# Kmatsuo57/cell-image-analysis

Hardware: AMD Instinct MI355X
Metric: cells/sec screened (CAE fwd + recon-MSE + SVM score), 64x64 (higher is better)
Workload: dtype f32 (results in the fp32 error class; the contractions run as split 16-bit products on the matrix pipe, fp32 accumulate: conv1..conv6 as 2 fp16 terms x 3 products with exact power-of-two scales from each cell's own data, the PCA GEMM as 3 bf16 terms x 6 products, conv7's 32 -> 16 channel contraction; 1 GPU; BASELINE.json configs[2]: screening inference, 1000000 synthetic 64x64 crops on one GPU, resident in HBM, CAE fwd + recon MSE/MAE + RobustScaler + PCA(100) + 2x OCSVM score on device; cells_per_gpu=1000000, global_cells=1000000, chunk_cells=65536, detector_train_cells=5000, weights=random init (Glorot, non-trivial BN), seed 42, parallelism=dp1

## Files before the change

cell-image-analysis_amd/csrc/api.hip:

```cpp
#include "api_internal.hpp"
#include "tensor_archive.hpp"

using namespace cs;

static thread_local std::string g_err;

namespace cs {
int fail(int code, const char* fmt, ...)
{
    char buf[1024];
    va_list ap;
    va_start(ap, fmt);
    vsnprintf(buf, sizeof buf, fmt, ap);
    va_end(ap);
    g_err = buf;
    return code;
}
const char* last_error_cstr() { return g_err.c_str(); }
}

static const char* kKernelNames[K_COUNT] = {"conv1_relu_bn_pool", "conv2_relu_bn_pool", "conv3_relu_bn_pool",
                                            "conv4_relu_bn",      "conv5_up_relu_bn",   "conv6_up_relu_bn",
                                            "conv7_up_sigmoid_err", "scaler_pca",       "ocsvm_decision",
                                            "finalize",           "synth_crops",        "conv6_conv7_fused_err",
// ... 177 lines not shown
{
    std::vector<float> tmp;
    for (int l = 0; l < count; ++l) {
        const int cin = l == 0 ? 1 : kRefChannels[l - 1], cout = kRefChannels[l];
        const bool folded = (l == 4 || l == 5);
        const size_t nf = folded ? pack_conv_fragments_folded(cin, cout, nullptr, nullptr) : pack_conv_fragments(cin, cout, nullptr, nullptr);
        tmp.resize(nf);
        if (folded) pack_conv_fragments_folded(cin, cout, w->kernel[l], tmp.data());
        else pack_conv_fragments(cin, cout, w->kernel[l], tmp.data());
        int rc = upload(set.wfrag[l], tmp.data(), nf * sizeof(float));
        if (rc) return rc;
        std::vector<float> ep(3 * cout);
        for (int c = 0; c < cout; ++c) {
            const float s = w->bn_gamma[l][c] / sqrtf(w->bn_var[l][c] + w->bn_eps);
            ep[c] = w->bias[l][c];
            ep[cout + c] = s;
            ep[2 * cout + c] = w->bn_beta[l][c] - w->bn_mean[l][c] * s;
        }
        rc = upload(set.ep[l], ep.data(), ep.size() * sizeof(float));
        if (rc) return rc;
        if (l == 4 || l == 5) {
            tmp.resize(pack_wino_up_fragments(l, nullptr, nullptr));
            pack_wino_up_fragments(l, w->kernel[l], tmp.data());
            rc = upload(set.winoup[l], tmp.data(), tmp.size() * sizeof(float));
            if (rc) return rc;
        }
        if (l == 1 || l == 2) {
            tmp.resize(pack_wino_cs_fragments(l, nullptr, nullptr));
            pack_wino_cs_fragments(l, w->kernel[l], tmp.data());
            rc = upload(set.winocs[l], tmp.data(), tmp.size() * sizeof(float));
            if (rc) return rc;
        }
        if (l == 2) {
            std::vector<uint16_t> h2(pack_wino3_h2(nullptr, nullptr, nullptr));
            pack_wino3_h2(w->kernel[l], h2.data(), &set.c3h2_inv);
            rc = upload(set.c3h2, h2.data(), h2.size() * sizeof(uint16_t));
            if (rc) return rc;
        }
        if (l == 3) {
            std::vector<uint16_t> h2(pack_conv4_f16x2(nullptr, nullptr, nullptr));
            pack_conv4_f16x2(w->kernel[l], h2.data(), &set.c4h2_inv);
            rc = upload(set.c4h2, h2.data(), h2.size() * sizeof(uint16_t));
            if (rc) return rc;
        }
        if (l == 4) {
            std::vector<float> weff(pack_generic_folded(cin, cout, nullptr, nullptr));
            pack_generic_folded(cin, cout, w->kernel[l], weff.data());
            std::vector<uint16_t> h2(pack_conv5_f16x2(nullptr, nullptr, nullptr));
            pack_conv5_f16x2(weff.data(), h2.data(), &set.c5h2_inv);
            rc = upload(set.c5h2, h2.data(), h2.size() * sizeof(uint16_t));
            if (rc) return rc;
        }
        if (l == 5) {
            std::vector<float> weff(pack_generic_folded(cin, cout, nullptr, nullptr));
            pack_generic_folded(cin, cout, w->kernel[l], weff.data());
            std::vector<uint16_t> h2(pack_conv6_f16x2(nullptr, nullptr, nullptr));
            pack_conv6_f16x2(weff.data(), h2.data(), &set.c6h2_inv);
            rc = upload(set.c6h2, h2.data(), h2.size() * sizeof(uint16_t));
            if (rc) return rc;
        }
        if (l == 0) {
            tmp.resize(pack_conv12_conv1_fragments(nullptr, nullptr, nullptr));
            pack_conv12_conv1_fragments(w->kernel[l], ep.data() + cout, tmp.data());
            rc = upload(set.c12w1, tmp.data(), tmp.size() * sizeof(float));
            if (rc) return rc;
            pack_conv12_p1_bound(w->kernel[l], ep.data(), &set.p1a, &set.p1b);
            std::vector<unsigned int> wh(pack_conv12_conv1_h2(nullptr, nullptr, nullptr, nullptr));
            pack_conv12_conv1_h2(w->kernel[l], ep.data() + cout, wh.data(), &set.c12w1h2_inv);
            rc = upload(set.c12w1h2, wh.data(), wh.size() * sizeof(unsigned int));
            if (rc) return rc;
        }
        if (l == 1) {
            tmp.resize(pack_conv12_fragments(nullptr, nullptr, nullptr));
            pack_conv12_fragments(w->kernel[l], ep.data() + cout, tmp.data());
            rc = upload(set.c12, tmp.data(), tmp.size() * sizeof(float));
            if (rc) return rc;
            std::vector<unsigned int> uh(pack_conv12_fragments_h2(nullptr, nullptr, nullptr, nullptr));
            pack_conv12_fragments_h2(w->kernel[l], ep.data() + cout, uh.data(), &set.c12h2_inv);
            rc = upload(set.c12h2, uh.data(), uh.size() * sizeof(unsigned int));
            if (rc) return rc;
        }
    }
    set.n = count;
    return CS_OK;
}

static int pack_generic(GenSet& set, const cs_cae_weights* w, const Arch& a, int count, bool split16)
{
    for (int l = 0; l < count; ++l) {
        const int cin = a.cin(l), cout = a.ch[l];
        int rc = upload(set.w[l], w->kernel[l], sizeof(float) * 9 * cin * cout);
        if (rc) return rc;
        set.folded[l] = l > a.n_enc && ((l < a.n_conv - 1 && conv_generic_folds(a.gh[l], a.gw[l], cin, cout)) ||
                                        (l == a.n_conv - 1 && cout == 1 && cin % 4 == 0));
        if (set.folded[l]) {
            std::vector<float> wf(pack_generic_folded(cin, cout, nullptr, nullptr));
            pack_generic_folded(cin, cout, w->kernel[l], wf.data());
            if ((rc = upload(set.wf[l], wf.data(), wf.size() * sizeof(float)))) return rc;
            if (split16 && l == a.n_conv - 1 && cout == 1 && conv_last_x3_takes(a.gh[l], a.gw[l], cin)) {
                std::vector<uint16_t> pl(pack_last_bf16x3(cin, nullptr, nullptr));
                pack_last_bf16x3(cin, wf.data(), pl.data());
                if ((rc = upload(set.wx3[l], pl.data(), pl.size() * sizeof(uint16_t)))) return rc;
                set.x3[l] = true;
            }
            if (split16 && l < a.n_conv - 1 && conv_generic_x3_takes(a.gh[l], a.gw[l], cin, cout, 1)) {
                std::vector<uint16_t> pl(pack_generic_bf16x3(16, cin, cout, nullptr, nullptr));
                pack_generic_bf16x3(16, cin, cout, wf.data(), pl.data());
                if ((rc = upload(set.wx3[l], pl.data(), pl.size() * sizeof(uint16_t)))) return rc;
                set.x3[l] = true;
                std::vector<uint16_t> ph(pack_generic_f16x2(16, cin, cout, nullptr, nullptr, nullptr));
// ... 922 lines not shown
        else if (k == K_SCALER_PCA) per_cell = 2.0 * (double)m->F * m->C;
        else if (k == K_SVM) per_cell = 0.0;
        *flops = per_cell * (double)m->prof_cells[k];
    }
    return CS_OK;
}

int cs_profile_mfma_per_cell(cs_model* m, int k, double* mfma)
{
    if (!m || !mfma || k < 0 || k >= K_COUNT) return fail(CS_ERR_INVALID, "bad kernel id");
    double v = 0.0;
    if (k == K_SCALER_PCA) {
        *mfma = m->has_det && !m->split16 ? (double)m->fpad * m->cpad / 1024.0 : 0.0;
        return CS_OK;
    }
    if (m->arch.ref) {
        const bool h2 = m->split16;
        switch (k) {
            case K_CONV1: v = 1536; break;
            case K_CONV2: v = 8192; break;
            case K_CONV3: v = h2 ? 0 : 2048; break;
            case K_CONV4: v = h2 ? 0 : 576; break;
            case K_CONV5: v = h2 ? 0 : 1152; break;
            case K_CONV6: v = 4608; break;
            case K_CONV67_FUSED: v = h2 ? 512 : 4608 + 512; break;
            case K_CONV12_FUSED: v = h2 ? 0 : 4608 + 1536 + 48; break;
            default: v = 0.0;
        }
    } else if (k <= K_CONV6 || k == K_CONV7_ERR) {
        const int l = k == K_CONV7_ERR ? m->arch.n_conv - 1 : k - K_CONV1;
        if (l < m->arch.n_conv && !(m->split16 && m->gae.x3[l])) {
            const int cout_pad = (m->arch.ch[l] + 15) / 16 * 16;
            v = (double)m->arch.gh[l] * m->arch.gw[l] / 16.0 * (cout_pad / 16) * (9.0 * m->arch.cin(l) / 4.0);
        }
    }
    *mfma = v;
    return CS_OK;
}

int cs_profile_bf16_mfma_per_cell(cs_model* m, int k, double* mfma)
{
    if (!m || !mfma || k < 0 || k >= K_COUNT) return fail(CS_ERR_INVALID, "bad kernel id");
    double v = 0.0;
    if (!m->split16) { *mfma = 0.0; return CS_OK; }
    if (k == K_SCALER_PCA && m->has_det) {
        *mfma = (double)(m->cpad / 16) * (m->fpad / 32) * 6.0 / 16.0;
        return CS_OK;
    }
    if (m->arch.ref) {
        if (k == K_CONV4) v = 4 * 2 * 9 * 3;
        if (k == K_CONV3) v = 16.0 * 4 * 2 * 2 * 3;
        if (k == K_CONV12_FUSED) v = 66 * 8 * 2 + 36 * 4 * 4 * 3;
        if (k == K_CONV5) v = 4 * 4 * 4 * 4 * 3 + (m->fuse45 ? 4 * 2 * 9 * 3 : 0);
        if (k == K_CONV67_FUSED) v = 4.0 * 16 * 2 * 4 * 2 * 3;
    } else if (k <= K_CONV6) {
        const int l = k - K_CONV1;
        if (l < m->arch.n_conv && m->gae.x3[l]) {
            const int cout_pad = (m->arch.ch[l] + 15) / 16 * 16;
            const double taps = l > m->arch.n_enc ? 4.0 : 9.0;
            const bool last = l == m->arch.n_conv - 1;
            v = (double)m->arch.gh[l] * m->arch.gw[l] / 16.0 * (cout_pad / 16) * taps * (m->arch.cin(l) / 32.0) * ((m->gae.h2_inv[l] != 0.0f && !last) ? 3.0 : 6.0);
        }
    }
    *mfma = v;
    return CS_OK;
}

}
```

cell-image-analysis_amd/csrc/common.hpp:

```cpp
#pragma once
#include <hip/hip_runtime.h>
#include <stdint.h>
#include <stdio.h>

#include "../../include/cellscreen.h"

namespace cs {

typedef float f32x4 __attribute__((ext_vector_type(4)));

__device__ __forceinline__ unsigned int f16x2_split_word_scaled(float x, float S)
{
    unsigned int pk;
    asm("v_fma_mixlo_f16 %0, %1, %2, 0\n\t"
        "v_fma_mixhi_f16 %0, %1, %2, -%0 op_sel:[0,0,0] op_sel_hi:[0,0,1]"
        : "=&v"(pk) : "v"(x), "v"(S));
    return pk;
}
__device__ __forceinline__ void f16x2_split6_exchange(const float (&v)[6], unsigned int sel, unsigned int (&out)[6])
{
    unsigned int p0, p1, p2, p3, p4, p5;
    asm("v_cvt_f16_f32 %6, %12\n\t"
        "v_cvt_f16_f32 %7, %13\n\t"
        "v_cvt_f16_f32 %8, %14\n\t"
// ... 18 lines not shown
        "v_perm_b32 %3, %3, %9, %18\n\t"
        "v_perm_b32 %4, %4, %10, %18\n\t"
        "v_perm_b32 %5, %5, %11, %18"
        : "=&v"(out[0]), "=&v"(out[1]), "=&v"(out[2]), "=&v"(out[3]), "=&v"(out[4]), "=&v"(out[5]),
          "=&v"(p0), "=&v"(p1), "=&v"(p2), "=&v"(p3), "=&v"(p4), "=&v"(p5)
        : "v"(v[0]), "v"(v[1]), "v"(v[2]), "v"(v[3]), "v"(v[4]), "v"(v[5]), "v"(sel));
}

struct LayerGeom {
    int H, W, cin, cout;
    bool pool;
    bool ups;
    bool last;
};

enum KernelId {
    K_CONV1 = 0, K_CONV2, K_CONV3, K_CONV4, K_CONV5, K_CONV6, K_CONV7_ERR,
    K_SCALER_PCA, K_SVM, K_FINALIZE, K_SYNTH, K_CONV67_FUSED, K_CONV12_FUSED, K_COUNT
};

hipError_t launch_conv_mfma(int layer, const float* in, const float* wfrag, const float* ep,
                            float* out, int64_t n_cells, hipStream_t stream, bool folded = false);
size_t pack_conv_fragments_folded(int cin, int cout, const float* hwio, float* dst);
hipError_t launch_conv_wino_cs(int layer, const float* in, const float* ufrag, const float* ep, float* out, int64_t n_cells,
                               hipStream_t stream);
size_t pack_wino_cs_fragments(int layer, const float* hwio, float* dst);
hipError_t launch_conv3_wino_h2(const float* in, const uint16_t* uplanes, float inv_sw, const float* ep, float* out, int64_t n_cells,
                                hipStream_t stream);
size_t pack_wino3_h2(const float* hwio, uint16_t* dst, float* inv_sw);
hipError_t launch_conv12_fused(const float* x, const float* w1frag, const float* ep1, const float* ufrag, const float* ep2, float* p2,
                               int64_t n_cells, hipStream_t stream, const unsigned int* ufrag_h2 = nullptr,
                               float p1a = 0.0f, float p1b = 0.0f, float inv_sw = 1.0f, const unsigned int* w1h2 = nullptr, float inv_sw1 = 1.0f);
size_t pack_conv12_conv1_h2(const float* hwio, const float* bn_scale, unsigned int* dst, float* inv_sw1);
size_t pack_conv12_fragments_h2(const float* hwio, const float* bn_scale, unsigned int* dst, float* inv_sw);
void pack_conv12_p1_bound(const float* hwio1, const float* ep1, float* a1, float* b1);
size_t pack_conv12_fragments(const float* hwio, const float* bn_scale, float* dst);
size_t pack_conv12_conv1_fragments(const float* hwio, const float* bn_scale, float* dst);
hipError_t launch_conv4_h2(const float* in, const uint16_t* wfrag, float inv_sw, const float* ep, float* out, int64_t n_cells, hipStream_t stream);
size_t pack_conv4_f16x2(const float* hwio, uint16_t* dst, float* inv_sw);
hipError_t launch_conv5_h2(const float* in, const uint16_t* wfrag, float inv_sw, const float* ep, float* out, int64_t n_cells, hipStream_t stream);
hipError_t launch_conv45_h2(const float* in, const uint16_t* w4, float inv_sw4, const float* ep4, const uint16_t* w5, float inv_sw5,
                            const float* ep5, float* out, int64_t n_cells, hipStream_t stream);
size_t pack_conv5_f16x2(const float* weff, uint16_t* dst, float* inv_sw);
hipError_t launch_conv_wino_up(int layer, const float* in, const float* ufrag, const float* ep, float* out, int64_t n_cells,
                               hipStream_t stream);
size_t pack_wino_up_fragments(int layer, const float* hwio, float* dst);
size_t pack_conv_fragments(int cin, int cout, const float* hwio, float* dst);

hipError_t launch_conv67_fused(const float* a5, const float* ufrag, const float* ep, const float* x, const float* weff_dev,
                               const float* b7_dev, float* errpart, int64_t n_cells, hipStream_t stream);
int conv67_fused_nparts();
hipError_t launch_conv67_h2(const float* a5, const uint16_t* wplanes, float inv_sw, const float* ep, const float* x, const float* weff_dev,
                            const float* b7_dev, float* errpart, int64_t n_cells, hipStream_t stream);
size_t pack_conv6_f16x2(const float* weff, uint16_t* dst, float* inv_sw);
float f16x2_weight_scale(const float* w, size_t n);
void f16x2_split(float w, float S, uint16_t& hi, uint16_t& lo);

hipError_t launch_conv7_err(const float* a6, const float* x, const float* weff_dev, const float* b7_dev,
                            float* errpart, float* recon, int64_t n_cells, hipStream_t stream);
hipError_t launch_conv7_err_train(const float* a6, const float* x, const float* weff_dev, const float* b7_dev, float* errpart,
                                  float* recon, float* dz, float* dzsum_part, int64_t n_cells, hipStream_t stream);
void conv7_effective_weights(const float* w7_hwio, float* weff);

constexpr int TRAIN_MAX_PARTS = 256;
constexpr int BN_MAX_PARTS = 1024;
struct ReduceDesc { long dst; long len; const float* src; int nparts; long stride; };
hipError_t launch_conv_train_fwd(int layer, const float* in, const float* wfrag, const float* bias,
                                 float* relu_out, int64_t n_cells, hipStream_t stream, float* stats_part = nullptr,
                                 int* stats_parts = nullptr);
hipError_t launch_conv_dgrad(int layer, const float* dz, const float* wfrag_t, float* dx, int64_t n_cells,
                             hipStream_t stream);
hipError_t launch_bn_stats(const float* r, long P, int C, float* part, int* G, hipStream_t s);
hipError_t launch_bn_stats_final(const float* part, int G, int C, float eps, float momentum, float* mov_mean,
                                 float* mov_var, float* stats, hipStream_t s);
hipError_t launch_bn_stats_merge(const float* part, int G, int C, float* out , hipStream_t s);
hipError_t launch_bn_apply(const float* r, int C, const float* gamma, const float* beta, const float* stats, float* a,
                           long N, int H, int W, int pool, hipStream_t s);
hipError_t launch_loss_dz(const float* out, const float* y, long total, float* dz, float* dzsum_part, int* G, hipStream_t s,
                          const float* errpart = nullptr, long nparts = 0, float* out2 = nullptr);
hipError_t launch_loss_scalar(const float* errpart, long nparts, long nelem, float* out2, hipStream_t s);
hipError_t launch_bn_bwd_reduce(const float* da, const float* r, const float* stats, const float* gamma, const float* beta,
                                long N, int H, int W, int C, int pool, float* part, int* G, hipStream_t s);
hipError_t launch_bn_bwd_final(const float* part, int G, int C, double nred, float* sums, float* dgamma, float* dbeta,
                               hipStream_t s);
hipError_t launch_bn_bwd_dz(const float* da, const float* r, const float* stats, const float* gamma, const float* beta,
                            const float* sums, long N, int H, int W, int C, int pool, float* dz, float* dzsum_part,
                            int* Gz, hipStream_t s);
hipError_t launch_wgrad(int layer, const float* xin, const float* dz, float* part, int64_t n_cells, int* nparts,
                        hipStream_t s);
hipError_t launch_reduce_all(const ReduceDesc* descs_dev, int ndesc, long total_len, float* flat_grad, hipStream_t s,
                             const float* errpart = nullptr, long nparts = 0, long nelem = 0, float* out2 = nullptr);
hipError_t launch_adam(float* p, const float* g, float* m, float* v, long n, float alpha, float b1, float b2, float eps, hipStream_t s,
                       const float* batch_scal, double* macc);
enum { GEN_EPI_BN = 0, GEN_EPI_BN_POOL = 1, GEN_EPI_SIGMOID = 2, GEN_EPI_RELU = 3, GEN_EPI_PLAIN = 4 };
int conv_generic_supported(int H, int W, int cin, int cout, char* why, size_t why_len);
hipError_t launch_conv_generic(const float* in, const float* w_hwio, const float* ep, float* out, int64_t n, int H, int W, int cin,
                               int cout, int ups, int epi, hipStream_t stream, const float* w_folded = nullptr);
size_t pack_generic_folded(int cin, int cout, const float* hwio, float* dst);
int conv_generic_x3_takes(int H, int W, int cin, int cout, int ups);
size_t pack_generic_bf16x3(int ntaps, int cin, int cout, const float* w, uint16_t* dst);
hipError_t launch_pack_generic_bf16x3(const float* w, int ntaps, int cin, int cout, uint16_t* dst, hipStream_t stream);
hipError_t launch_conv_generic_x3(const float* in, const uint16_t* wplanes, const float* ep, float* out, int64_t n, int H, int W, int cin,
                                  int cout, int ups, int epi, hipStream_t stream, float inv_sw = 0.0f);
size_t pack_generic_f16x2(int ntaps, int cin, int cout, const float* w, uint16_t* dst, float* inv_sw);
int conv_last_x3_takes(int H, int W, int cin);
size_t pack_last_bf16x3(int cin, const float* weff, uint16_t* dst);
hipError_t launch_conv_last_x3(const float* in, const uint16_t* wplanes, const float* ep, float* out, int64_t n, int H, int W, int cin,
// ... 48 lines not shown
```

cell-image-analysis_amd/csrc/conv_wino_up.hip:

```cpp
#include "common.hpp"

#include <type_traits>

#include <cmath>
#include <cstdlib>
#include <cstring>

namespace cs {

namespace {

template <int HS_, int WS_, int CIN_, int COUT_>
struct WUCfg {
    static constexpr int HS = HS_, WS = WS_, CIN = CIN_, COUT = COUT_;
    static constexpr int HO = 2 * HS, WO = 2 * WS;
    static constexpr int TW = WS / 2;
    static constexpr int SR = 2 * (16 / TW);
    static constexpr int R = SR + 2, WP = WS + 2;
    static constexpr int PS = CIN + 4;
    static constexpr int STRIP = R * WP * PS * 4;
    static constexpr int LDS = 2 * STRIP;
    static constexpr int NGRP = HS / SR;
    static constexpr int NQ = CIN / 16, KS = CIN / 4;
    static constexpr int NSW = COUT / 32;
    static constexpr int NB = 9 * KS * NSW;
    static constexpr int C4 = CIN / 4, TOT = R * WP * C4;
    static constexpr int THREADS = 512;
    static constexpr int EPR = WS * C4;
    static constexpr int RPP = THREADS / EPR;
    static constexpr int NLD = (R + RPP - 1) / RPP;
    static_assert(THREADS % EPR == 0 && (EPR & (EPR - 1)) == 0 && (C4 & (C4 - 1)) == 0, "row-wise staging");
    static_assert(NB == 144 && LDS <= 160 * 1024 && HS % SR == 0 && (NSW == 1 || NSW == 2), "layer does not fit this design");
};
using WUL6 = WUCfg<16, 16, 64, 32>;
using WUL5 = WUCfg<8, 8, 32, 64>;

template <class C>
__device__ __forceinline__ f32x4 wu_load(const float* __restrict__ cellp, int y0, int j, int rsub, int goff)
{
    int sy = y0 - 1 + rsub + C::RPP * j;
    sy = sy < 0 ? 0 : (sy > C::HS - 1 ? C::HS - 1 : sy);
    return *(const f32x4*)(cellp + sy * (C::WS * C::CIN) + goff);
}
template <class C>
__device__ __forceinline__ void wu_store(float* strip, int y0, int j, int rsub, int loff, f32x4 v)
{
    const int r = rsub + C::RPP * j;
    const int sy = y0 - 1 + r;
    if (sy < 0 || sy >= C::HS) v = f32x4{0.0f, 0.0f, 0.0f, 0.0f};
    if (C::R % C::RPP == 0 || r < C::R) *(f32x4*)(strip + r * (C::WP * C::PS) + loff) = v;
}

__device__ __forceinline__ unsigned long long wu_stamp()
{
    unsigned long long t;
    __builtin_amdgcn_sched_barrier(0);
    asm volatile("s_memtime %0\n\ts_waitcnt lgkmcnt(0)" : "=s"(t)::"memory");
    __builtin_amdgcn_sched_barrier(0);
    return t;
// ... 322 lines not shown
                if (y == 0) { ta0 = 0.0f; ta1 = 0.0f; }
                const float v = ((ta0 + ta1) + (tb0 + tb1)) + b7;
                const float rr = f67_sigmoid(v);
                const float d = xv[h] - rr;
                s2 = fmaf(d, d, s2);
                s1 += fabsf(d);
            }
            if (grp == C::NGRP - 1 && wave == 0) {
                const int nb = (2 + px) * 4;
                const float* ra = tb + ((31 & (F67::TSLOTS - 1)) * F67::TWD + xh) * 16 + nb;
                const float v = (ra[0] + ra[16 + 1]) + b7;
                const float rr = f67_sigmoid(v);
                const float d = xtail - rr;
                s2 = fmaf(d, d, s2);
                s1 += fabsf(d);
            }
            if constexpr (DIAG) {
                asm volatile("" ::"v"(s2), "v"(s1));
                const unsigned long long t = wu_stamp(); dg[4] += t - dt; dt = t;
            }
            buf ^= 1;
        }
#pragma unroll
        for (int off = 32; off > 0; off >>= 1) {
            s2 += __shfl_down(s2, off, 64);
            s1 += __shfl_down(s1, off, 64);
        }
        if (lane == 0) {
            errpart[((size_t)cell * F67::NPARTS + wave) * 2 + 0] = s2;
            errpart[((size_t)cell * F67::NPARTS + wave) * 2 + 1] = s1;
        }
    }
    if constexpr (DIAG) {
        if (lane == 0) {
#pragma unroll
            for (int k = 0; k < 5; ++k) diag[((size_t)blockIdx.x * 8 + wave) * 5 + k] = dg[k];
        }
    }
}

struct F67T {
    static constexpr int TW = 36;
    static constexpr int T_BYTES = F67::TSLOTS * 16 * TW * 4;
};

typedef _Float16 f16x8 __attribute__((ext_vector_type(8)));
typedef _Float16 f16x4 __attribute__((ext_vector_type(4)));

struct F67H {
    static constexpr int PLB = 2 * 64;
    static constexpr int PXB = 2 * PLB + 32;
    static constexpr int ROWB = 18 * PXB;
    static constexpr int STRIP = 6 * ROWB;
    static constexpr int TW = F67T::TW;
    static constexpr int T_BYTES = F67T::T_BYTES;
    static constexpr int PA = 40;
    static constexpr int A6_BYTES = 8 * 32 * PA * 4;
    static constexpr int WP = 40;
    static constexpr int W_BYTES = 16 * WP * 4;
    static constexpr int OFF_MAX = STRIP + A6_BYTES + T_BYTES + W_BYTES;
    static constexpr int LDS = OFF_MAX + 16;
    static_assert(LDS <= 160 * 1024 && STRIP % 16 == 0, "LDS budget");
};

__device__ __forceinline__ unsigned int h2_rowmax(unsigned int m)
{
    unsigned int o;
    o = (unsigned int)__builtin_amdgcn_update_dpp(0, (int)m, 0xB1, 0xF, 0xF, true);  m = m > o ? m : o;
    o = (unsigned int)__builtin_amdgcn_update_dpp(0, (int)m, 0x4E, 0xF, 0xF, true);  m = m > o ? m : o;
    o = (unsigned int)__builtin_amdgcn_update_dpp(0, (int)m, 0x124, 0xF, 0xF, true); m = m > o ? m : o;
    o = (unsigned int)__builtin_amdgcn_update_dpp(0, (int)m, 0x128, 0xF, 0xF, true); m = m > o ? m : o;
    return m;
}

__device__ __forceinline__ void h2_scale(unsigned int mbits, float& S, float& invS)
{
    int E = (int)((mbits >> 23) & 0xffu);
    E = E < 40 ? 40 : (E > 254 ? 254 : E);
    S = __builtin_bit_cast(float, (unsigned int)(268 - E) << 23);
    invS = __builtin_bit_cast(float, (unsigned int)(E - 14) << 23);
}

__device__ __forceinline__ void h2_split4(const f32x4& x, float S, f16x4& hi, f16x4& lo)
{
    const f32x4 v = x * S;
    hi = __builtin_convertvector(v, f16x4);
    const f32x4 r = v - __builtin_convertvector(hi, f32x4);
    lo = __builtin_convertvector(r, f16x4);
}

__device__ __forceinline__ void h2_store(char* strip, int j, int rsub, int loffb, const f32x4& v, float S)
{
    const int r = rsub + WUL6::RPP * j;
    f16x4 hi, lo;
    h2_split4(v, S, hi, lo);
    char* d = strip + r * F67H::ROWB + loffb;
    *(f16x4*)d = hi;
    *(f16x4*)(d + F67H::PLB) = lo;
}

__device__ __forceinline__ f32x4 h2_prep(int y0, int j, int rsub, f32x4 v, unsigned int& mx)
{
    const int sy = y0 - 1 + rsub + WUL6::RPP * j;
    if (sy < 0 || sy >= WUL6::HS) v = f32x4{0.0f, 0.0f, 0.0f, 0.0f};
    const float a = v[0], b = v[1], c = v[2], d = v[3];
    const unsigned int u = __builtin_bit_cast(unsigned int, fmaxf(fmaxf(fabsf(a), fabsf(b)), fmaxf(fabsf(c), fabsf(d))));
    mx = mx > u ? mx : u;
    return v;
}

template <bool DIAG>
__global__ __launch_bounds__(WUL6::THREADS, 2) void conv67_h2_kernel(
    const float* __restrict__ in , const f16x8* __restrict__ wfrag, const float* __restrict__ ep ,
    const float* __restrict__ x , const float* __restrict__ weff ,
    const float* __restrict__ b7p, float* __restrict__ errpart , long n_cells, float inv_sw,
    unsigned long long* __restrict__ diag)
{
    using C = WUL6;
    static_assert(C::NLD == 3 && C::RPP == 2 && C::R == 6 && C::EPR == 256, "row-wise staging constants");
    unsigned long long dg[5] = {0, 0, 0, 0, 0}, dt = 0;
    extern __shared__ __attribute__((aligned(16))) char smem[];
    float* a6s = (float*)(smem + F67H::STRIP);
    float* tb = (float*)(smem + F67H::STRIP + F67H::A6_BYTES);
    float* wl = (float*)(smem + F67H::STRIP + F67H::A6_BYTES + F67H::T_BYTES);
    unsigned int* mxw = (unsigned int*)(smem + F67H::OFF_MAX);
    const int tid = threadIdx.x, lane = tid & 63;
    const int wave = __builtin_amdgcn_readfirstlane(tid >> 6);
    const int ph = wave >> 1, wsl = wave & 1;
    const int pa = ph >> 1, pb = ph & 1;
    const int li = lane & 15, kq = lane >> 4;

    f16x8 B[4][2][2];
#pragma unroll
    for (int t = 0; t < 4; ++t)
#pragma unroll
        for (int k = 0; k < 2; ++k)
#pragma unroll
            for (int p = 0; p < 2; ++p) B[t][k][p] = wfrag[(((wave * 4 + t) * 2 + k) * 2 + p) * 64 + lane];
    const int co = wsl * 16 + li;
    const int cosw = co ^ ((kq & 1) << 4);
    const float bias = ep[co], bns = ep[C::COUT + co], bnt = ep[2 * C::COUT + co];
    const float b7 = b7p[0];

    const long first = blockIdx.x;
    if (first >= n_cells) return;
    const int se = tid & (C::EPR - 1), rsub = tid / C::EPR;
    const int spx = se / C::C4, sc4 = se & (C::C4 - 1);
    const int goff = spx * C::CIN + sc4 * 4;
    const int loffb = (spx + 1) * F67H::PXB + sc4 * 8;
    auto cell_ptr = [&](long cell) { return in + (size_t)cell * C::HS * C::WS * C::CIN; };
    for (int i = tid; i < F67H::LDS / 16; i += C::THREADS) ((f32x4*)smem)[i] = f32x4{0.0f, 0.0f, 0.0f, 0.0f};
    __syncthreads();
    wl[(tid >> 5) * F67H::WP + (tid & 31)] = weff[tid];
    float unscale;
    {
        f32x4 stg[C::NLD];
        unsigned int mx = 0;
#pragma unroll
        for (int j = 0; j < C::NLD; ++j) stg[j] = h2_prep(0, j, rsub, wu_load<C>(cell_ptr(first), 0, j, rsub, goff), mx);
        mx = h2_rowmax(mx);
        if (li == 0) atomicMax(&mxw[0], mx);
        __syncthreads();
        float S, invS;
        h2_scale(mxw[0], S, invS);
        unscale = invS * inv_sw;
#pragma unroll
        for (int j = 0; j < C::NLD; ++j) h2_store(smem, j, rsub, loffb, stg[j], S);
    }
    __syncthreads();
    if (tid == 0) mxw[0] = 0;
    const char* abase = smem + (pa * 18 + li + pb) * F67H::PXB + kq * 16;

    int strip_no = 0;
    for (long cell = first; cell < n_cells; cell += gridDim.x) {
        const float* xc = x + (size_t)cell * 64 * 64;
        float s2 = 0.0f, s1 = 0.0f;
#pragma unroll 1
        for (int grp = 0; grp < C::NGRP; ++grp) {
            const long ncell = grp < C::NGRP - 1 ? cell : cell + gridDim.x;
            const int ngrp = grp < C::NGRP - 1 ? grp + 1 : 0;
            const bool has_next = ncell < n_cells;
            ++strip_no;
            unsigned int* const mword = mxw + (strip_no & 1);

            if constexpr (DIAG) dt = wu_stamp();
            f32x4 stg[C::NLD];
            if (has_next) {
#pragma unroll
                for (int j = 0; j < C::NLD; ++j) stg[j] = wu_load<C>(cell_ptr(ncell), ngrp * C::SR, j, rsub, goff);
            }
            float xv[2];
#pragma unroll
            for (int h = 0; h < 2; ++h) {
                const int k = wave + 8 * h, o = 2 * (8 * grp + (k >> 1)) - 1 + (k & 1);
                xv[h] = xc[(o < 0 ? 0 : o) * 64 + lane];
            }
            float xtail = 0.0f;
            if (grp == C::NGRP - 1 && wave == 0) xtail = xc[63 * 64 + lane];

            if constexpr (DIAG) { const unsigned long long t = wu_stamp(); dg[0] += t - dt; dt = t; }
            f32x4 ah[4], al[4];
#pragma unroll
            for (int t = 0; t < 4; ++t) ah[t] = al[t] = f32x4{0.0f, 0.0f, 0.0f, 0.0f};
            auto rd = [&](int f, f16x8 (&a)[2]) {
                const int sr = f >> 2, rx = (f >> 1) & 1, k = f & 1;
                const char* p = abase + sr * F67H::ROWB + rx * F67H::PXB + k * 64;
                a[0] = *(const f16x8*)p;
                a[1] = *(const f16x8*)(p + F67H::PLB);
            };
            auto mac3 = [&](const f16x8 (&a)[2], const f16x8 (&b)[2], f32x4& dh, f32x4& dl) {
                dl = __builtin_amdgcn_mfma_f32_16x16x32_f16(a[0], b[1], dl, 0, 0, 0);
                dh = __builtin_amdgcn_mfma_f32_16x16x32_f16(a[0], b[0], dh, 0, 0, 0);
                dl = __builtin_amdgcn_mfma_f32_16x16x32_f16(a[1], b[0], dl, 0, 0, 0);
            };
            {
                f16x8 a[2];
                rd(0, a);
                __builtin_amdgcn_sched_group_barrier(0x100, 2, 0);
#pragma unroll
                for (int f = 0; f < 20; ++f) {
                    const int sr = f >> 2, rx = (f >> 1) & 1, k = f & 1;
                    f16x8 an[2] = {a[0], a[1]};
                    if (f + 1 < 20) rd(f + 1, an);
                    if (sr < 4) mac3(a, B[rx][k], ah[sr], al[sr]);
                    if (sr > 0) mac3(a, B[2 + rx][k], ah[sr - 1], al[sr - 1]);
                    a[0] = an[0]; a[1] = an[1];
                    __builtin_amdgcn_sched_group_barrier(0x100, 2, 0);
                    if (sr > 0 && sr < 4) __builtin_amdgcn_sched_group_barrier(0x008, 6, 0);
                    else __builtin_amdgcn_sched_group_barrier(0x008, 3, 0);
                }
            }
            if constexpr (DIAG) {
                asm volatile("" ::"v"(ah[0][0]), "v"(al[3][3]));
                const unsigned long long t = wu_stamp(); dg[1] += t - dt; dt = t;
            }
#pragma unroll
            for (int t = 0; t < 4; ++t)
#pragma unroll
                for (int r = 0; r < 4; ++r) {
                    const float v = fmaxf(fmaf(ah[t][r] + al[t][r], unscale, bias), 0.0f);
                    a6s[((2 * t + pa) * 32 + 2 * (4 * kq + r) + pb) * F67H::PA + cosw] = fmaf(v, bns, bnt);
                }
            if (has_next) {
                unsigned int mx = 0;
#pragma unroll
                for (int j = 0; j < C::NLD; ++j) stg[j] = h2_prep(ngrp * C::SR, j, rsub, stg[j], mx);
                mx = h2_rowmax(mx);
                if (li == 0) atomicMax(mword, mx);
            }
            __syncthreads();
            if constexpr (DIAG) { const unsigned long long t = wu_stamp(); dg[2] += t - dt; dt = t; }
            {
                const int wrow = 4 * ((li >> 3) | (((li >> 2) & 1) << 1)) + (li & 3);
                float wc[8];
                *(f32x4*)&wc[0] = *(const f32x4*)(wl + wrow * F67H::WP + 4 * kq);
                *(f32x4*)&wc[4] = *(const f32x4*)(wl + wrow * F67H::WP + 4 * kq + 16);
                const int pix = 4 * (li & 3) + (li >> 2), sw = ((li >> 1) & 1) << 4;
                const float* ap = a6s + (wave * 32 + pix) * F67H::PA + 4 * kq;
                const f32x4 a00 = *(const f32x4*)(ap + sw), a01 = *(const f32x4*)(ap + (sw ^ 16));
                const f32x4 a10 = *(const f32x4*)(ap + 16 * F67H::PA + sw), a11 = *(const f32x4*)(ap + 16 * F67H::PA + (sw ^ 16));
                f32x4 t0 = f32x4{0.0f, 0.0f, 0.0f, 0.0f}, t1 = t0;
#pragma unroll
                for (int s = 0; s < 4; ++s) {
                    t0 = __builtin_amdgcn_mfma_f32_16x16x4f32(wc[s], a00[s], t0, 0, 0, 0);
                    t1 = __builtin_amdgcn_mfma_f32_16x16x4f32(wc[s], a10[s], t1, 0, 0, 0);
                }
#pragma unroll
                for (int s = 0; s < 4; ++s) {
                    t0 = __builtin_amdgcn_mfma_f32_16x16x4f32(wc[4 + s], a01[s], t0, 0, 0, 0);
                    t1 = __builtin_amdgcn_mfma_f32_16x16x4f32(wc[4 + s], a11[s], t1, 0, 0, 0);
                }
                const int rblk = kq == 0 ? 0 : (kq == 1 ? 3 : (kq == 2 ? 1 : 2));
                float* tw = tb + ((((8 * grp + wave) & (F67::TSLOTS - 1)) * 16) + 4 * rblk) * F67H::TW + pix + 1 - (kq >> 1);
#pragma unroll
                for (int r = 0; r < 4; ++r) { tw[r * F67H::TW] = t0[r]; tw[r * F67H::TW + 16] = t1[r]; }
            }
            if (has_next) {
                float S, invS;
                h2_scale(*mword, S, invS);
                unscale = invS * inv_sw;
#pragma unroll
                for (int j = 0; j < C::NLD; ++j) h2_store(smem, j, rsub, loffb, stg[j], S);
            }
            __syncthreads();
            if (tid == 0) *mword = 0;
            if constexpr (DIAG) { const unsigned long long t = wu_stamp(); dg[3] += t - dt; dt = t; }
            const int px = lane & 1, xh = lane >> 1;
#pragma unroll
            for (int h = 0; h < 2; ++h) {
                const int k = wave + 8 * h;
                const int y = 8 * grp + (k >> 1), e = k & 1;
                if (2 * y - 1 + e < 0) continue;
                const int nb = (e ? px : 3 - px) * 4;
                const float* ra = tb + ((((y - 1) & (F67::TSLOTS - 1)) * 16) + nb) * F67H::TW + xh;
                const float* rb = tb + (((y & (F67::TSLOTS - 1)) * 16) + nb) * F67H::TW + xh;
                float ta0 = ra[0], ta1 = ra[F67H::TW + 1];
                const float tb0 = rb[2 * F67H::TW], tb1 = rb[3 * F67H::TW + 1];
                if (y == 0) { ta0 = 0.0f; ta1 = 0.0f; }
                const float v = ((ta0 + ta1) + (tb0 + tb1)) + b7;
                const float rr = f67_sigmoid(v);
                const float d = xv[h] - rr;
                s2 = fmaf(d, d, s2);
                s1 += fabsf(d);
            }
            if (grp == C::NGRP - 1 && wave == 0) {
                const int nb = (3 - px) * 4;
                const float* ra = tb + (((31 & (F67::TSLOTS - 1)) * 16) + nb) * F67H::TW + xh;
                const float v = (ra[0] + ra[F67H::TW + 1]) + b7;
                const float rr = f67_sigmoid(v);
                const float d = xtail - rr;
                s2 = fmaf(d, d, s2);
                s1 += fabsf(d);
            }
            if constexpr (DIAG) {
                asm volatile("" ::"v"(s2), "v"(s1));
                const unsigned long long t = wu_stamp(); dg[4] += t - dt; dt = t;
            }
        }
#pragma unroll
        for (int off = 32; off > 0; off >>= 1) {
            s2 += __shfl_down(s2, off, 64);
            s1 += __shfl_down(s1, off, 64);
        }
        if (lane == 0) {
            errpart[((size_t)cell * F67::NPARTS + wave) * 2 + 0] = s2;
            errpart[((size_t)cell * F67::NPARTS + wave) * 2 + 1] = s1;
        }
    }
    if constexpr (DIAG) {
        if (lane == 0) {
#pragma unroll
            for (int k = 0; k < 5; ++k) diag[((size_t)blockIdx.x * 8 + wave) * 5 + k] = dg[k];
        }
    }
}
// ... 67 lines not shown

}

int conv67_fused_nparts() { return F67::NPARTS; }

hipError_t launch_conv67_fused(const float* a5, const float* ufrag, const float* ep, const float* x, const float* weff_dev,
                               const float* b7_dev, float* errpart, int64_t n_cells, hipStream_t stream)
{
    static int cus = 0;
    static const bool diag = getenv("CS_WINO_DIAG") != nullptr;
    if (!cus) {
        hipError_t e = hipFuncSetAttribute((const void*)conv67_fused_kernel<false>, hipFuncAttributeMaxDynamicSharedMemorySize, F67::LDS);
        if (e != hipSuccess) return e;
        e = hipFuncSetAttribute((const void*)conv67_fused_kernel<true>, hipFuncAttributeMaxDynamicSharedMemorySize, F67::LDS);
        if (e != hipSuccess) return e;
        int dev = 0;
        if ((e = hipGetDevice(&dev)) != hipSuccess) return e;
        if ((e = hipDeviceGetAttribute(&cus, hipDeviceAttributeMultiprocessorCount, dev)) != hipSuccess) return e;
        if (diag && !g_wu_diag[3]) {
            if ((e = hipMalloc(&g_wu_diag[3], (size_t)cus * 40 * sizeof(unsigned long long))) != hipSuccess) return e;
            g_wu_diag_blocks[3] = cus;
        }
    }
    if (n_cells <= 0) return hipSuccess;
    const unsigned grid = (unsigned)(n_cells < cus ? n_cells : cus);
    if (diag)
        hipLaunchKernelGGL(conv67_fused_kernel<true>, dim3(grid), dim3(WUL6::THREADS), F67::LDS, stream, a5, ufrag, ep, x, weff_dev, b7_dev,
                           errpart, (long)n_cells, g_wu_diag[3]);
    else
        hipLaunchKernelGGL(conv67_fused_kernel<false>, dim3(grid), dim3(WUL6::THREADS), F67::LDS, stream, a5, ufrag, ep, x, weff_dev, b7_dev,
                           errpart, (long)n_cells, (unsigned long long*)nullptr);
    return hipGetLastError();
}

float f16x2_weight_scale(const float* w, size_t n)
{
    float m = 0.0f;
    for (size_t i = 0; i < n; ++i) m = fmaxf(m, fabsf(w[i]));
    if (!(m > 0.0f) || !std::isfinite(m)) return 1.0f;
    int e;
    frexpf(m, &e);
    return ldexpf(1.0f, 15 - e);
}

void f16x2_split(float w, float S, uint16_t& hi, uint16_t& lo)
{
    const float v = w * S;
    const _Float16 h = (_Float16)v;
    const _Float16 l = (_Float16)(v - (float)h);
    memcpy(&hi, &h, 2);
    memcpy(&lo, &l, 2);
}

size_t pack_conv6_f16x2(const float* weff, uint16_t* dst, float* inv_sw)
{
    const size_t n = (size_t)8 * 4 * 2 * 2 * 64 * 8;
    if (!dst) return n;
    const float S = f16x2_weight_scale(weff, (size_t)16 * 64 * 32);
    if (inv_sw) *inv_sw = 1.0f / S;
    for (int w = 0; w < 8; ++w)
        for (int t = 0; t < 4; ++t)
            for (int k = 0; k < 2; ++k)
                for (int l = 0; l < 64; ++l)
                    for (int j = 0; j < 8; ++j) {
                        const int ph = w >> 1, half = w & 1, li = l & 15, kq = l >> 4;
                        const float v = weff[((size_t)(ph * 4 + t) * 64 + 32 * k + 8 * kq + j) * 32 + 16 * half + li];
                        uint16_t pl[2];
                        f16x2_split(v, S, pl[0], pl[1]);
                        for (int p = 0; p < 2; ++p) dst[((((((size_t)w * 4 + t) * 2 + k) * 2 + p) * 64) + l) * 8 + j] = pl[p];
                    }
    return n;
}

hipError_t launch_conv67_h2(const float* a5, const uint16_t* wplanes, float inv_sw, const float* ep, const float* x, const float* weff_dev,
                            const float* b7_dev, float* errpart, int64_t n_cells, hipStream_t stream)
{
    static int cus = 0;
    static const bool diag = getenv("CS_WINO_DIAG") != nullptr;
    if (!cus) {
        hipError_t e = hipFuncSetAttribute((const void*)conv67_h2_kernel<false>, hipFuncAttributeMaxDynamicSharedMemorySize, F67H::LDS);
        if (e != hipSuccess) return e;
        e = hipFuncSetAttribute((const void*)conv67_h2_kernel<true>, hipFuncAttributeMaxDynamicSharedMemorySize, F67H::LDS);
        if (e != hipSuccess) return e;

        int dev = 0;
        if ((e = hipGetDevice(&dev)) != hipSuccess) return e;
        if ((e = hipDeviceGetAttribute(&cus, hipDeviceAttributeMultiprocessorCount, dev)) != hipSuccess) return e;
        if (diag && !g_wu_diag[3]) {
            if ((e = hipMalloc(&g_wu_diag[3], (size_t)cus * 40 * sizeof(unsigned long long))) != hipSuccess) return e;
            g_wu_diag_blocks[3] = cus;
        }
    }
    if (n_cells <= 0) return hipSuccess;
    const unsigned grid = (unsigned)(n_cells < cus ? n_cells : cus);
    if (diag)
        hipLaunchKernelGGL(conv67_h2_kernel<true>, dim3(grid), dim3(WUL6::THREADS), F67H::LDS, stream, a5, (const f16x8*)wplanes, ep, x,
                           weff_dev, b7_dev, errpart, (long)n_cells, inv_sw, g_wu_diag[3]);
    else
        hipLaunchKernelGGL(conv67_h2_kernel<false>, dim3(grid), dim3(WUL6::THREADS), F67H::LDS, stream, a5, (const f16x8*)wplanes, ep, x,
                           weff_dev, b7_dev, errpart, (long)n_cells, inv_sw, (unsigned long long*)nullptr);
    return hipGetLastError();
}

size_t pack_wino_up_fragments(int layer, const float* hwio, float* dst)
{
    return layer == 5 ? pack_frags<WUL6>(hwio, dst) : pack_frags<WUL5>(hwio, dst);
}

hipError_t launch_conv_wino_up(int layer, const float* in, const float* ufrag, const float* ep, float* out, int64_t n_cells,
                               hipStream_t stream)
{
    if (layer == 5) return launch<WUL6>(layer, in, ufrag, ep, out, n_cells, stream);
    if (layer == 4) return launch<WUL5>(layer, in, ufrag, ep, out, n_cells, stream);
    return hipErrorInvalidValue;
}

}

extern "C" int cs_debug_wino_up_diag(int layer, double out5[5])
{
    using namespace cs;
    if (layer < 3 || layer > 5 || !g_wu_diag[layer]) return -1;
    if (hipDeviceSynchronize() != hipSuccess) return -2;
// ... 10 lines not shown
```

Baseline: 5.526 million cells/s.

## Rewrite conv6 upsample contraction to share row taps across output row phases

Recasts the fused conv6 (upsample+conv) weights into three row-combination sets (minus, sum, plus) per column phase and stores a row-difference image of the input strip next to the strip in LDS. Each wave then computes two output row phases from shared products, combining them as 2*m+s and 2*p+s, so the matrix work per cell shrinks from 4 taps per phase to fewer shared taps. The costs are a second LDS image, an extra staged input row per thread, and differences that are rounded to fp16 at half scale, which can shift the error slightly.

```diff
diff --git a/cell-image-analysis_amd/csrc/api.hip b/cell-image-analysis_amd/csrc/api.hip
--- a/cell-image-analysis_amd/csrc/api.hip
+++ b/cell-image-analysis_amd/csrc/api.hip
@@ -253,10 +253,8 @@
             if (rc) return rc;
         }
         if (l == 5) {
-            std::vector<float> weff(pack_generic_folded(cin, cout, nullptr, nullptr));
-            pack_generic_folded(cin, cout, w->kernel[l], weff.data());
             std::vector<uint16_t> h2(pack_conv6_f16x2(nullptr, nullptr, nullptr));
-            pack_conv6_f16x2(weff.data(), h2.data(), &set.c6h2_inv);
+            pack_conv6_f16x2(w->kernel[l], h2.data(), &set.c6h2_inv);
             rc = upload(set.c6h2, h2.data(), h2.size() * sizeof(uint16_t));
             if (rc) return rc;
         }
@@ -1285,7 +1283,7 @@
         if (k == K_CONV3) v = 16.0 * 4 * 2 * 2 * 3;
         if (k == K_CONV12_FUSED) v = 66 * 8 * 2 + 36 * 4 * 4 * 3;
         if (k == K_CONV5) v = 4 * 4 * 4 * 4 * 3 + (m->fuse45 ? 4 * 2 * 9 * 3 : 0);
-        if (k == K_CONV67_FUSED) v = 4.0 * 16 * 2 * 4 * 2 * 3;
+        if (k == K_CONV67_FUSED) v = 16.0 * 2 * 2 * 3 * 2 * 2 * 3;
     } else if (k <= K_CONV6) {
         const int l = k - K_CONV1;
         if (l < m->arch.n_conv && m->gae.x3[l]) {
diff --git a/cell-image-analysis_amd/csrc/common.hpp b/cell-image-analysis_amd/csrc/common.hpp
--- a/cell-image-analysis_amd/csrc/common.hpp
+++ b/cell-image-analysis_amd/csrc/common.hpp
@@ -94,7 +94,7 @@
 int conv67_fused_nparts();
 hipError_t launch_conv67_h2(const float* a5, const uint16_t* wplanes, float inv_sw, const float* ep, const float* x, const float* weff_dev,
                             const float* b7_dev, float* errpart, int64_t n_cells, hipStream_t stream);
-size_t pack_conv6_f16x2(const float* weff, uint16_t* dst, float* inv_sw);
+size_t pack_conv6_f16x2(const float* hwio, uint16_t* dst, float* inv_sw);
 float f16x2_weight_scale(const float* w, size_t n);
 void f16x2_split(float w, float S, uint16_t& hi, uint16_t& lo);
 
diff --git a/cell-image-analysis_amd/csrc/conv_wino_up.hip b/cell-image-analysis_amd/csrc/conv_wino_up.hip
--- a/cell-image-analysis_amd/csrc/conv_wino_up.hip
+++ b/cell-image-analysis_amd/csrc/conv_wino_up.hip
@@ -5,6 +5,7 @@
 #include <cmath>
 #include <cstdlib>
 #include <cstring>
+#include <vector>
 
 namespace cs {
 
@@ -433,15 +434,19 @@
     static constexpr int PXB = 2 * PLB + 32;
     static constexpr int ROWB = 18 * PXB;
     static constexpr int STRIP = 6 * ROWB;
+    static constexpr int DSTRIP = 5 * ROWB;
+    static constexpr int OFF_A6 = STRIP + DSTRIP;
     static constexpr int TW = F67T::TW;
     static constexpr int T_BYTES = F67T::T_BYTES;
     static constexpr int PA = 40;
     static constexpr int A6_BYTES = 8 * 32 * PA * 4;
     static constexpr int WP = 40;
     static constexpr int W_BYTES = 16 * WP * 4;
-    static constexpr int OFF_MAX = STRIP + A6_BYTES + T_BYTES + W_BYTES;
+    static constexpr int OFF_T = OFF_A6 + A6_BYTES;
+    static constexpr int OFF_W = OFF_T + T_BYTES;
+    static constexpr int OFF_MAX = OFF_W + W_BYTES;
     static constexpr int LDS = OFF_MAX + 16;
-    static_assert(LDS <= 160 * 1024 && STRIP % 16 == 0, "LDS budget");
+    static_assert(LDS <= 160 * 1024 && STRIP % 128 == 0 && OFF_A6 % 16 == 0, "LDS budget; the D image sits on the strip's banks");
 };
 
 __device__ __forceinline__ unsigned int h2_rowmax(unsigned int m)
@@ -470,19 +475,35 @@
     lo = __builtin_convertvector(r, f16x4);
 }
 
-__device__ __forceinline__ void h2_store(char* strip, int j, int rsub, int loffb, const f32x4& v, float S)
-{
-    const int r = rsub + WUL6::RPP * j;
+__device__ __forceinline__ f32x4 h2_load(const float* __restrict__ cellp, int y0, int r, int goff)
+{
+    int sy = y0 - 1 + r;
+    sy = sy < 0 ? 0 : (sy > WUL6::HS - 1 ? WUL6::HS - 1 : sy);
+    return *(const f32x4*)(cellp + sy * (WUL6::WS * WUL6::CIN) + goff);
+}
+
+__device__ __forceinline__ void h2_store(char* img, int r, int loffb, const f32x4& v, float S)
+{
     f16x4 hi, lo;
     h2_split4(v, S, hi, lo);
-    char* d = strip + r * F67H::ROWB + loffb;
+    char* d = img + r * F67H::ROWB + loffb;
     *(f16x4*)d = hi;
     *(f16x4*)(d + F67H::PLB) = lo;
 }
 
-__device__ __forceinline__ f32x4 h2_prep(int y0, int j, int rsub, f32x4 v, unsigned int& mx)
-{
-    const int sy = y0 - 1 + rsub + WUL6::RPP * j;
+__device__ __forceinline__ void h2_store_strip(char* smem, int rsub, int loffb, const f32x4 (&stg)[4], float S)
+{
+    const float Sd = 0.5f * S;
+    if (rsub == 0) { h2_store(smem, 1, loffb, stg[1], S); h2_store(smem, 2, loffb, stg[2], S); }
+    else { h2_store(smem, 3, loffb, stg[0], S); h2_store(smem, 4, loffb, stg[1], S); }
+#pragma unroll
+    for (int j = 0; j < 2; ++j) h2_store(smem + F67H::STRIP, 3 * rsub + j, loffb, stg[j + 1] - stg[j], Sd);
+    if (rsub == 0) h2_store(smem + F67H::STRIP, 2, loffb, stg[3] - stg[2], Sd);
+}
+
+__device__ __forceinline__ f32x4 h2_prep(int y0, int r, f32x4 v, unsigned int& mx)
+{
+    const int sy = y0 - 1 + r;
     if (sy < 0 || sy >= WUL6::HS) v = f32x4{0.0f, 0.0f, 0.0f, 0.0f};
     const float a = v[0], b = v[1], c = v[2], d = v[3];
     const unsigned int u = __builtin_bit_cast(unsigned int, fmaxf(fmaxf(fabsf(a), fabsf(b)), fmaxf(fabsf(c), fabsf(d))));
@@ -498,26 +519,27 @@
     unsigned long long* __restrict__ diag)
 {
     using C = WUL6;
-    static_assert(C::NLD == 3 && C::RPP == 2 && C::R == 6 && C::EPR == 256, "row-wise staging constants");
+    static_assert(C::R == 6 && C::EPR == 256 && C::THREADS == 2 * C::EPR, "staging: two halves of the workgroup, three adjacent rows each");
     unsigned long long dg[5] = {0, 0, 0, 0, 0}, dt = 0;
     extern __shared__ __attribute__((aligned(16))) char smem[];
-    float* a6s = (float*)(smem + F67H::STRIP);
-    float* tb = (float*)(smem + F67H::STRIP + F67H::A6_BYTES);
-    float* wl = (float*)(smem + F67H::STRIP + F67H::A6_BYTES + F67H::T_BYTES);
+    float* a6s = (float*)(smem + F67H::OFF_A6);
+    float* tb = (float*)(smem + F67H::OFF_T);
+    float* wl = (float*)(smem + F67H::OFF_W);
     unsigned int* mxw = (unsigned int*)(smem + F67H::OFF_MAX);
     const int tid = threadIdx.x, lane = tid & 63;
     const int wave = __builtin_amdgcn_readfirstlane(tid >> 6);
-    const int ph = wave >> 1, wsl = wave & 1;
-    const int pa = ph >> 1, pb = ph & 1;
+    const int pb = wave >> 2, wsl = (wave >> 1) & 1, rp = wave & 1;
     const int li = lane & 15, kq = lane >> 4;
 
-    f16x8 B[4][2][2];
-#pragma unroll
-    for (int t = 0; t < 4; ++t)
-#pragma unroll
-        for (int k = 0; k < 2; ++k)
-#pragma unroll
-            for (int p = 0; p < 2; ++p) B[t][k][p] = wfrag[(((wave * 4 + t) * 2 + k) * 2 + p) * 64 + lane];
+    f16x8 B[3][2][2][2];
+#pragma unroll
+    for (int t = 0; t < 3; ++t)
+#pragma unroll
+        for (int rx = 0; rx < 2; ++rx)
+#pragma unroll
+            for (int k = 0; k < 2; ++k)
+#pragma unroll
+                for (int p = 0; p < 2; ++p) B[t][rx][k][p] = wfrag[(((((wave >> 1) * 3 + t) * 2 + rx) * 2 + k) * 2 + p) * 64 + lane];
     const int co = wsl * 16 + li;
     const int cosw = co ^ ((kq & 1) << 4);
     const float bias = ep[co], bns = ep[C::COUT + co], bnt = ep[2 * C::COUT + co];
@@ -525,7 +547,7 @@
 
     const long first = blockIdx.x;
     if (first >= n_cells) return;
-    const int se = tid & (C::EPR - 1), rsub = tid / C::EPR;
+    const int se = tid & (C::EPR - 1), rsub = wave >> 2;
     const int spx = se / C::C4, sc4 = se & (C::C4 - 1);
     const int goff = spx * C::CIN + sc4 * 4;
     const int loffb = (spx + 1) * F67H::PXB + sc4 * 8;
@@ -535,22 +557,23 @@
     wl[(tid >> 5) * F67H::WP + (tid & 31)] = weff[tid];
     float unscale;
     {
-        f32x4 stg[C::NLD];
+        f32x4 stg[4];
         unsigned int mx = 0;
 #pragma unroll
-        for (int j = 0; j < C::NLD; ++j) stg[j] = h2_prep(0, j, rsub, wu_load<C>(cell_ptr(first), 0, j, rsub, goff), mx);
+        for (int j = 0; j < 3; ++j) stg[j] = h2_prep(0, 3 * rsub + j, h2_load(cell_ptr(first), 0, 3 * rsub + j, goff), mx);
+        stg[3] = h2_load(cell_ptr(first), 0, 3, goff);
         mx = h2_rowmax(mx);
         if (li == 0) atomicMax(&mxw[0], mx);
         __syncthreads();
         float S, invS;
         h2_scale(mxw[0], S, invS);
         unscale = invS * inv_sw;
-#pragma unroll
-        for (int j = 0; j < C::NLD; ++j) h2_store(smem, j, rsub, loffb, stg[j], S);
+        h2_store_strip(smem, rsub, loffb, stg, S);
     }
     __syncthreads();
     if (tid == 0) mxw[0] = 0;
-    const char* abase = smem + (pa * 18 + li + pb) * F67H::PXB + kq * 16;
+    const char* rbase = smem + ((2 * rp + 1) * 18 + li + pb) * F67H::PXB + kq * 16;
+    const char* dbase = smem + F67H::STRIP + (2 * rp * 18 + li + pb) * F67H::PXB + kq * 16;
 
     int strip_no = 0;
     for (long cell = first; cell < n_cells; cell += gridDim.x) {
@@ -565,10 +588,11 @@
             unsigned int* const mword = mxw + (strip_no & 1);
 
             if constexpr (DIAG) dt = wu_stamp();
-            f32x4 stg[C::NLD];
+            f32x4 stg[4];
             if (has_next) {
 #pragma unroll
-                for (int j = 0; j < C::NLD; ++j) stg[j] = wu_load<C>(cell_ptr(ncell), ngrp * C::SR, j, rsub, goff);
+                for (int j = 0; j < 3; ++j) stg[j] = h2_load(cell_ptr(ncell), ngrp * C::SR, 3 * rsub + j, goff);
+                stg[3] = h2_load(cell_ptr(ncell), ngrp * C::SR, 3, goff);
             }
             float xv[2];
 #pragma unroll
@@ -580,19 +604,21 @@
             if (grp == C::NGRP - 1 && wave == 0) xtail = xc[63 * 64 + lane];
 
             if constexpr (DIAG) { const unsigned long long t = wu_stamp(); dg[0] += t - dt; dt = t; }
-            f32x4 ah[4], al[4];
-#pragma unroll
-            for (int t = 0; t < 4; ++t) ah[t] = al[t] = f32x4{0.0f, 0.0f, 0.0f, 0.0f};
+            f32x4 am[2][2], as[2][2], ap[2][2];
+#pragma unroll
+            for (int i = 0; i < 2; ++i)
+#pragma unroll
+                for (int h = 0; h < 2; ++h) am[i][h] = as[i][h] = ap[i][h] = f32x4{0.0f, 0.0f, 0.0f, 0.0f};
             auto rd = [&](int f, f16x8 (&a)[2]) {
-                const int sr = f >> 2, rx = (f >> 1) & 1, k = f & 1;
-                const char* p = abase + sr * F67H::ROWB + rx * F67H::PXB + k * 64;
+                const int c = f / 5, q = f % 5, rx = c >> 1, k = c & 1;
+                const char* p = ((q & 1) ? rbase : dbase) + (q >> 1) * F67H::ROWB + rx * F67H::PXB + k * 64;
                 a[0] = *(const f16x8*)p;
                 a[1] = *(const f16x8*)(p + F67H::PLB);
             };
-            auto mac3 = [&](const f16x8 (&a)[2], const f16x8 (&b)[2], f32x4& dh, f32x4& dl) {
-                dl = __builtin_amdgcn_mfma_f32_16x16x32_f16(a[0], b[1], dl, 0, 0, 0);
-                dh = __builtin_amdgcn_mfma_f32_16x16x32_f16(a[0], b[0], dh, 0, 0, 0);
-                dl = __builtin_amdgcn_mfma_f32_16x16x32_f16(a[1], b[0], dl, 0, 0, 0);
+            auto mac3 = [&](const f16x8 (&a)[2], const f16x8 (&b)[2], f32x4 (&d)[2]) {
+                d[1] = __builtin_amdgcn_mfma_f32_16x16x32_f16(a[0], b[1], d[1], 0, 0, 0);
+                d[0] = __builtin_amdgcn_mfma_f32_16x16x32_f16(a[0], b[0], d[0], 0, 0, 0);
+                d[1] = __builtin_amdgcn_mfma_f32_16x16x32_f16(a[1], b[0], d[1], 0, 0, 0);
             };
             {
                 f16x8 a[2];
@@ -600,32 +626,39 @@
                 __builtin_amdgcn_sched_group_barrier(0x100, 2, 0);
 #pragma unroll
                 for (int f = 0; f < 20; ++f) {
-                    const int sr = f >> 2, rx = (f >> 1) & 1, k = f & 1;
+                    const int c = f / 5, q = f % 5, rx = c >> 1, k = c & 1;
                     f16x8 an[2] = {a[0], a[1]};
                     if (f + 1 < 20) rd(f + 1, an);
-                    if (sr < 4) mac3(a, B[rx][k], ah[sr], al[sr]);
-                    if (sr > 0) mac3(a, B[2 + rx][k], ah[sr - 1], al[sr - 1]);
+                    if (q == 0) mac3(a, B[0][rx][k], am[0]);
+                    if (q == 1) mac3(a, B[1][rx][k], as[0]);
+                    if (q == 2) { mac3(a, B[2][rx][k], ap[0]); mac3(a, B[0][rx][k], am[1]); }
+                    if (q == 3) mac3(a, B[1][rx][k], as[1]);
+                    if (q == 4) mac3(a, B[2][rx][k], ap[1]);
                     a[0] = an[0]; a[1] = an[1];
                     __builtin_amdgcn_sched_group_barrier(0x100, 2, 0);
-                    if (sr > 0 && sr < 4) __builtin_amdgcn_sched_group_barrier(0x008, 6, 0);
+                    if (q == 2) __builtin_amdgcn_sched_group_barrier(0x008, 6, 0);
                     else __builtin_amdgcn_sched_group_barrier(0x008, 3, 0);
                 }
             }
             if constexpr (DIAG) {
-                asm volatile("" ::"v"(ah[0][0]), "v"(al[3][3]));
+                asm volatile("" ::"v"(am[0][0][0]), "v"(ap[1][1][3]));
                 const unsigned long long t = wu_stamp(); dg[1] += t - dt; dt = t;
             }
-#pragma unroll
-            for (int t = 0; t < 4; ++t)
+            auto post = [&](float v) { v = fmaxf(fmaf(v, unscale, bias), 0.0f); return fmaf(v, bns, bnt); };
+#pragma unroll
+            for (int i = 0; i < 2; ++i)
 #pragma unroll
                 for (int r = 0; r < 4; ++r) {
-                    const float v = fmaxf(fmaf(ah[t][r] + al[t][r], unscale, bias), 0.0f);
-                    a6s[((2 * t + pa) * 32 + 2 * (4 * kq + r) + pb) * F67H::PA + cosw] = fmaf(v, bns, bnt);
+                    const float sv = as[i][0][r] + as[i][1][r];
+                    const float v0 = fmaf(am[i][0][r] + am[i][1][r], 2.0f, sv), v1 = fmaf(ap[i][0][r] + ap[i][1][r], 2.0f, sv);
+                    float* o = a6s + ((2 * (2 * rp + i)) * 32 + 2 * (4 * kq + r) + pb) * F67H::PA + cosw;
+                    o[0] = post(v0);
+                    o[32 * F67H::PA] = post(v1);
                 }
             if (has_next) {
                 unsigned int mx = 0;
 #pragma unroll
-                for (int j = 0; j < C::NLD; ++j) stg[j] = h2_prep(ngrp * C::SR, j, rsub, stg[j], mx);
+                for (int j = 0; j < 3; ++j) stg[j] = h2_prep(ngrp * C::SR, 3 * rsub + j, stg[j], mx);
                 mx = h2_rowmax(mx);
                 if (li == 0) atomicMax(mword, mx);
             }
@@ -660,8 +693,7 @@
                 float S, invS;
                 h2_scale(*mword, S, invS);
                 unscale = invS * inv_sw;
-#pragma unroll
-                for (int j = 0; j < C::NLD; ++j) h2_store(smem, j, rsub, loffb, stg[j], S);
+                h2_store_strip(smem, rsub, loffb, stg, S);
             }
             __syncthreads();
             if (tid == 0) *mword = 0;
@@ -835,23 +867,36 @@
     memcpy(&lo, &l, 2);
 }
 
-size_t pack_conv6_f16x2(const float* weff, uint16_t* dst, float* inv_sw)
-{
-    const size_t n = (size_t)8 * 4 * 2 * 2 * 64 * 8;
+size_t pack_conv6_f16x2(const float* hwio, uint16_t* dst, float* inv_sw)
+{
+    const size_t n = (size_t)4 * 3 * 2 * 2 * 2 * 64 * 8;
     if (!dst) return n;
-    const float S = f16x2_weight_scale(weff, (size_t)16 * 64 * 32);
+    std::vector<float> sets((size_t)2 * 2 * 3 * 64 * 32);
+    for (int b = 0; b < 2; ++b)
+        for (int rx = 0; rx < 2; ++rx)
+            for (int ci = 0; ci < 64; ++ci)
+                for (int co = 0; co < 32; ++co) {
+                    double A[3] = {0.0, 0.0, 0.0};
+                    for (int dy = -1; dy <= 1; ++dy)
+                        for (int dx = -1; dx <= 1; ++dx)
+                            if (((b + dx) >> 1) == b + rx - 1) A[dy + 1] += (double)hwio[((size_t)((dy + 1) * 3 + (dx + 1)) * 64 + ci) * 32 + co];
+                    const double v[3] = {-A[0], A[0] + A[1] + A[2], A[2]};
+                    for (int t = 0; t < 3; ++t) sets[((((size_t)b * 2 + rx) * 3 + t) * 64 + ci) * 32 + co] = (float)v[t];
+                }
+    const float S = f16x2_weight_scale(sets.data(), sets.size());
     if (inv_sw) *inv_sw = 1.0f / S;
-    for (int w = 0; w < 8; ++w)
-        for (int t = 0; t < 4; ++t)
-            for (int k = 0; k < 2; ++k)
-                for (int l = 0; l < 64; ++l)
-                    for (int j = 0; j < 8; ++j) {
-                        const int ph = w >> 1, half = w & 1, li = l & 15, kq = l >> 4;
-                        const float v = weff[((size_t)(ph * 4 + t) * 64 + 32 * k + 8 * kq + j) * 32 + 16 * half + li];
-                        uint16_t pl[2];
-                        f16x2_split(v, S, pl[0], pl[1]);
-                        for (int p = 0; p < 2; ++p) dst[((((((size_t)w * 4 + t) * 2 + k) * 2 + p) * 64) + l) * 8 + j] = pl[p];
-                    }
+    for (int w = 0; w < 4; ++w)
+        for (int t = 0; t < 3; ++t)
+            for (int rx = 0; rx < 2; ++rx)
+                for (int k = 0; k < 2; ++k)
+                    for (int l = 0; l < 64; ++l)
+                        for (int j = 0; j < 8; ++j) {
+                            const int b = w >> 1, half = w & 1, li = l & 15, kq = l >> 4;
+                            const float v = sets[((((size_t)b * 2 + rx) * 3 + t) * 64 + 32 * k + 8 * kq + j) * 32 + 16 * half + li];
+                            uint16_t pl[2];
+                            f16x2_split(v, S, pl[0], pl[1]);
+                            for (int p = 0; p < 2; ++p) dst[(((((((size_t)w * 3 + t) * 2 + rx) * 2 + k) * 2 + p) * 64) + l) * 8 + j] = pl[p];
+                        }
     return n;
 }
 
```

Result: no change. 5.525 million cells/s (-0.0%).
